# yazdayy/sound-event-detection

Measured on AMD Instinct MI355X. Metric: 10s@16kHz clips/sec (whole node) + ms/clip p50, Cnn_9_Gru_FrameAtt logmel, higher is better.
Workload: dtype f32 (conv2 of block 1 as Winograd F(4x4,3x3), blocks 2-4 as Winograd F(4x4,3x3): f32 transforms, f32 MFMA, f32 accumulate)

## Files before the change

sound-event-detection_amd/csrc/api.cpp:

```cpp
#include <new>
#include <hip/hip_runtime.h>

#include <algorithm>
#include <cmath>
#include <complex>
#include <cstdarg>
#include <cstdio>
#include <cstdlib>
#include <cstring>
#include <map>
#include <mutex>
#include <string>
#include <vector>

#include "../../include/sedx.h"
#include "rank.h"
#include "sedx_internal.h"

using namespace sedx;

struct EvSet {
  hipEvent_t ev[SEDX_N_STAGES + 1] = {};
  bool rec[SEDX_N_STAGES + 1] = {};
};
// ... 204 lines not shown
}

sedx_status run_body(sedx_handle* h, const ForwardPlan& p, float* ws, float* d_fw, float* d_clip, float* d_emb,
                     hipStream_t s) {
  const DevWeights& w = h->w;
  const Tuning& t = h->tune;
  const Geometry& g = p.g;
  const int64_t B = p.B;
  const int iB = (int)B, M = p.M, T3 = (int)g.Ts;
  float* X0 = ws + p.x0.off;
  float* A = ws + p.A.off;
  int* sched = reinterpret_cast<int*>(ws + p.sched.off);
  mark(h, 12, s);
  auto block1_first = [&]() {
    switch (p.block1) {
      case B1_CONV1C4_F43: launch_conv1_c4(X0, iB, (int)g.T, w.c1_w, w.c1_b, A, s); break;
      case B1_CONV1_F23:
      case B1_CONV1_F43: launch_conv1_nhwc(X0, iB, (int)g.T, w.c1_w, w.c1_b, A, s); break;
      case B1_PAD_EXACT:
      case B1_PAD_X3: launch_pad_x0(X0, iB, (int)g.T, A, s); break;
      case B1_F23_FUSED: break;
      case B1_VGG: launch_vgg_conv1(X0, iB, (int)g.T, w.c1_w, w.c1_b, A, s); break;
    }
  };
  if (p.claims) HIP_TRY(h, hipMemsetAsync(sched, 0, 7 * CONV_SCHED_INTS * sizeof(int), s));
  const bool first_early = t.pipelined && t.pipe_conv1_first;
  if (first_early) block1_first();
  if (t.pipelined && h->conv_done_recorded) HIP_TRY(h, hipStreamWaitEvent(s, h->conv_done, 0));
  mark(h, 1, s);
  capture(h, 0, X0, (size_t)B * g.T * 64, s);
  if (!first_early) block1_first();
// ... 19 lines not shown
      launch_conv3x3_deep(in, iB, c.T, c.F, c.cin, c.cout, w.wp[7] + deep_w_off(l), w.cb[7] + deep_b_off(l), out,
                          c.epi, p.c4 && l == 0, s);
      capture(h, i < 7 ? 2 + i : 40 + (i - 7), out, (size_t)B * c.To * c.Fo * c.cout, s);
      continue;
    }
    int* claim = p.claims ? sched + i * CONV_SCHED_INTS : nullptr;
    mark(h, 2 + i, s);
    WinoFamily wf;
    const bool wino = conv_launch_family(p, i, &wf);
    if (wino && wf == WINO_F23_BLOCK1)
      launch_block1_wino(in, iB, c.T, w.c1_w, w.c1_b, w.wu[k], w.cb[k], out, w.zero, w.trash, s, p.c4);
    else if (wino && wf == WINO_F23)
      launch_conv3x3_wino(in, iB, c.T, c.F, c.cin, c.cout, w.wu[k], w.cb[k], out, c.epi, w.zero, w.trash, s, c.order);
    else if (wino)
      launch_conv3x3_wino43(in, iB, c.T, c.F, c.cin, c.cout, w.wu43[k], w.cb[k], out, c.epi, w.trash, s, c.order,
                            p.c4, 0, claim);
    else if (i == 0 && p.block1 == B1_PAD_X3)
      launch_block1_fused_x3(nullptr, iB, c.T, in, w.c1_wt, w.c1_b, w.wx3[k], w.cb[k], out, claim, s);
    else if (i == 0)
      launch_block1_exact(in, iB, c.T, w.c1_w, w.c1_b, w.wp[k], w.cb[k], out, w.zero, s);
    else if (p.family == CONV_X3)
      launch_conv3x3_x3(in, iB, c.T, c.F, c.cin, c.cout, w.wx3[k], w.cb[k], out, c.epi, claim, s);
    else
      launch_conv3x3(in, iB, c.T, c.F, c.cin, c.cout, w.wp[k], w.cb[k], out, c.epi, w.zero, s);
    if (p.c4 && c.epi != EPI_FMEAN)
      capture_c4(h, 2 + i, out, B, c.To, c.Fo, c.cout, s);
    else
      capture(h, 2 + i, out, (size_t)B * c.To * c.Fo * c.cout, s);
  }
  mark(h, 9, s);
  if (t.pipelined) {
// ... 142 lines not shown
  h->cap_buf = d_buf;
  h->cap_bytes = bytes;
  return SEDX_OK;
}

sedx_status sedx_set_tuning(sedx_handle* h, int32_t knob, int32_t value) {
  if (!h) return SEDX_EINVAL;
  static const struct {
    int knob, lo, hi;
    int Tuning::*field;
  } knobs[] = {{SEDX_TUNE_GRU_KERNEL, SEDX_GRU_KERNEL_COOP, SEDX_GRU_KERNEL_PAIR, &Tuning::gru_kernel},
               {SEDX_TUNE_GRU_HANDOFF, SEDX_GRU_HANDOFF_AUTO, SEDX_GRU_HANDOFF_LOCAL, &Tuning::gru_handoff},
               {SEDX_TUNE_WINO_BLOCK1, 0, 2, &Tuning::wino_block1},
               {SEDX_TUNE_MEL_MFMA, 0, 1, &Tuning::mel_mfma},
               {SEDX_TUNE_GRU_SPIN, 0, INT32_MAX, &Tuning::gru_spin},
               {SEDX_TUNE_WINO_ORDER, 0, 2, &Tuning::wino_order},
               {SEDX_TUNE_GAMMA_SPEC, 0, 1, &Tuning::gamma_spec},
               {SEDX_TUNE_WINO_F43, 0, 2, &Tuning::wino_f43}};
  for (const auto& k : knobs) {
    if (k.knob != knob) continue;
    if (value < k.lo || value > k.hi) return fail(h, SEDX_EINVAL, "bad value %d for tuning knob %d", (int)value, (int)knob);
    h->tune.*k.field = value;
    return SEDX_OK;
  }
  return fail(h, SEDX_EINVAL, "unknown tuning knob %d", (int)knob);
}

sedx_status sedx_check_error(sedx_handle* h) {
  if (!h) return SEDX_EINVAL;
  return check_async_error(h);
}
// ... 584 lines not shown
```

sound-event-detection_amd/csrc/conv_wino.hip:

```cpp
#include <type_traits>

#include "sedx_internal.h"
#include "wino_geom.h"

namespace sedx {

typedef float f32x16 __attribute__((ext_vector_type(16)));
typedef float f32x4w __attribute__((ext_vector_type(4)));

#ifndef SEDX_WINO_ABL
#define SEDX_WINO_ABL 0
#endif
#ifndef SEDX_WINO_C1MFMA
#define SEDX_WINO_C1MFMA 0
#endif
#ifndef SEDX_WINO_VG
#define SEDX_WINO_VG 3
#endif
#ifndef SEDX_WINO_VG1
#define SEDX_WINO_VG1 9
#endif
#ifdef SEDX_WINO_STAMPS
__device__ unsigned long long g_wino_stamps[16];
#define WS_DECL                                      \
// ... 733 lines not shown
#pragma unroll
      for (int k = 0; k < 9; ++k) acc = fmaf(xv[k], s_w[(4 * cc + c) * 9 + k], acc);
      y[c] = fmaxf(acc + s_b[4 * cc + c], 0.0f);
    }
    *reinterpret_cast<float4*>(ob + (int64_t)cc * T * 256) = make_float4(y[0], y[1], y[2], y[3]);
  }
}

void launch_conv1_c4(const float* x0, int B, int T, const float* w1, const float* b1, float* out, hipStream_t s) {
  const int rb = (T + C1_ROWS - 1) / C1_ROWS;
  const int64_t blocks = (int64_t)B * rb;
  if (B <= 0 || T <= 0 || blocks > INT32_MAX || (int64_t)T * 64 > INT32_MAX) return note_launch_error(hipErrorInvalidValue);
  hipLaunchKernelGGL(conv1_c4_kernel, dim3((unsigned)blocks), dim3(256), 0, s, x0, T, rb, w1, b1, out);
}

#ifdef SEDX_WINO_STAMPS
void wino_stamps_rw(unsigned long long* h, bool reset) {
  if (reset) {
    static const unsigned long long z[16] = {};
    (void)hipMemcpyToSymbol(HIP_SYMBOL(g_wino_stamps), z, sizeof(z));
  } else {
    (void)hipMemcpyFromSymbol(h, HIP_SYMBOL(g_wino_stamps), 16 * sizeof(unsigned long long));
  }
}
#endif


}
```

sound-event-detection_amd/csrc/conv_wino43.hip:

```cpp
#include <type_traits>

#include "sedx_internal.h"
#include "wino_geom.h"

namespace sedx {

typedef float w43_f32x4 __attribute__((ext_vector_type(4)));

#ifndef SEDX_W43_ABL
#define SEDX_W43_ABL 0
#endif
#ifndef SEDX_W43_PRIO
#define SEDX_W43_PRIO 2
#endif
#ifndef SEDX_W43_USEL
#define SEDX_W43_USEL 1
#endif
#ifndef SEDX_W43_DMA_SPLIT
#define SEDX_W43_DMA_SPLIT 5
#endif

#ifdef SEDX_W43_STAMPS
__device__ unsigned long long g_w43_stamps[8];
#define W43_MARK(i)                                            \
  {                                                            \
    const unsigned long long n_ = __builtin_amdgcn_s_memtime(); \
    w43_st[i] += n_ - w43_t;                                   \
    w43_t = n_;                                                \
  }
#else
#define W43_MARK(i)
#endif

template <int N>
// ... 26 lines not shown
  v[1] = a + b;
  v[2] = a - b;
  const float c = e[4] - e[2], t = e[3] - e[1];
  v[3] = fmaf(2.0f, t, c);
  v[4] = fmaf(-2.0f, t, c);
  v[5] = fmaf(4.0f, e[1], fmaf(-5.0f, e[3], e[5]));
}
__device__ __forceinline__ void w43_at(const float (&m)[6], float (&z)[4]) {
  const float s12 = m[1] + m[2], d12 = m[1] - m[2], s34 = m[3] + m[4], d34 = m[3] - m[4];
  z[0] = (m[0] + s12) + s34;
  z[1] = fmaf(2.0f, d34, d12);
  z[2] = fmaf(4.0f, s34, s12);
  z[3] = fmaf(8.0f, d34, d12) + m[5];
}

template <int F, int EPI, int ROW, bool C4, int NT, int TG>
__device__ __forceinline__ void w43_body(const float* __restrict__ in, int B, int T, int Cin, int Cout,
                                         const float* __restrict__ U, int u_bytes, const float* __restrict__ bias,
                                         float* __restrict__ out, float* __restrict__ trash, int tb_per_clip,
                                         int ngroups, int order2d, int* __restrict__ sched, int wv) {
  using G = W43Geom<F, TG>;
  constexpr int RS = G::RS, PS = G::PS;
  static_assert(TG == 2 || (NT == 1 && (F == 16 || F == 8)), "16-tile items: 16-channel, F = 16 / 8 only");
  static_assert(NT == 4 || NT == 1, "channel tiles per item");
  using UF = typename std::conditional<NT == 4, w43_f32x4, float>::type;
  constexpr int VM = NT == 4 ? G::VM : TG == 2 ? 5 : 6;
  extern __shared__ __attribute__((aligned(16))) float smem[];

  const int lane = (int)__builtin_amdgcn_mbcnt_hi(~0u, __builtin_amdgcn_mbcnt_lo(~0u, 0u));
  const int tg = TG == 2 ? wv & 1 : 0;
  const int kk = lane >> 4, nn = lane & 15;

  auto decode = [&](int item, int& b_, int& t0_, int& g_) -> bool {
    const int xcd = item & 7, j = item >> 3;
    int jb, cgi;
    if constexpr (NT == 1) {
      const int tbl = B * tb_per_clip, gi = j / tbl, tb = j - gi * tbl;
      g_ = 8 * gi + xcd;
      if (g_ >= ngroups) return false;
      b_ = tb / tb_per_clip;
      t0_ = 4 * G::TRW * (tb - b_ * tb_per_clip);
// ... 42 lines not shown
    item = __builtin_amdgcn_readfirstlane(cl[1]);
  }
  if (!decode(item, b, t0, grp)) {
    claim_done();
    return;
  }

  const int tr = (F == 16 ? 4 * tg : F == 8 ? 8 * tg : F == 64 ? tg : 0) + nn / G::TFG;
  const int tf = (F == 32 ? 4 * tg : 0) + nn % G::TFG;

  const __amdgpu_buffer_rsrc_t r_in =
      __builtin_amdgcn_make_buffer_rsrc((void*)in, 0, (int)((int64_t)B * T * F * Cin * 4), 0x00020000);
  const __amdgpu_buffer_rsrc_t r_u = __builtin_amdgcn_make_buffer_rsrc((void*)U, 0, u_bytes, 0x00020000);
  const int nchunks = Cin / 4;
  auto halo_off = [&](int b_, int t0_) -> uint32_t {
    const int q = 64 * wv + lane;
    const int row = q / RS, col = q - (q / RS) * RS;
    const int t = t0_ - 1 + row, f = col - 1;
    const bool ok = row < G::RT && col < G::CS && t >= 0 && t < T && f >= 0 && f < F;
    if constexpr (C4)
      return ok ? (uint32_t)((((b_ * (Cin / 4) * T + t) * F + f) * 16)) : 0x80000000u;
    return ok ? (uint32_t)((((b_ * T + t) * F + f) * Cin) * 4) : 0x80000000u;
  };
  const uint32_t u_voff = 16 * lane + 1024 * wv;
  const uint32_t u_voff1 = wv < 9 ? u_voff : 0x80000000u;
  const uint32_t u_voff2 = wv + 6 < 9 ? u_voff + 6144 : 0x80000000u;
  const uint32_t bytes_per_chunk_u = 4 * G::USZ;
  auto dma_u_units = [&](int g_, int cc, int uslot, auto q0_tag, auto q1_tag) {
    if constexpr (SEDX_W43_ABL & 2) return;
    constexpr int Q0 = decltype(q0_tag)::value, Q1 = decltype(q1_tag)::value;
// ... 6 lines not shown
        if constexpr (TG == 1) w43_dma16(u_voff2, r_u, so, m0 + 6144);
      }
      return;
    }
    const uint32_t so = __builtin_amdgcn_readfirstlane((uint32_t)((g_ * nchunks + cc) * bytes_per_chunk_u));
    const uint32_t m0 = __builtin_amdgcn_readfirstlane(w43_lds_addr(smem + G::U_OFF + uslot * G::USZ + 256 * wv));
#pragma unroll
    for (int q = Q0; q < Q1; ++q) w43_dma16(u_voff, r_u, so + q * 12288, m0 + q * 12288);
  };
  auto dma_u = [&](int g_, int cc, int uslot) {
    dma_u_units(g_, cc, uslot, std::integral_constant<int, 0>{}, std::integral_constant<int, 3>{});
  };
  auto dma_h_planes = [&](uint32_t hof, int cc, int hslot, auto p0_tag, auto p1_tag) {
    if constexpr (SEDX_W43_ABL & 1) return;
    constexpr int P0 = decltype(p0_tag)::value, P1 = decltype(p1_tag)::value;
    const uint32_t so = __builtin_amdgcn_readfirstlane((uint32_t)(16 * (C4 ? cc * T * F : cc)));
    const bool tw = wv == G::HB;
    const uint32_t m0 = __builtin_amdgcn_readfirstlane(
        w43_lds_addr(tw ? smem + G::HTRASH_OFF : smem + G::H_OFF + hslot * G::HALO + 64 * wv));
    const uint32_t pstep = tw ? 0u : 4u * PS;
#pragma unroll
    for (int q = P0; q < P1; ++q) w43_dma4(hof, r_in, so + 4 * q, m0 + q * pstep);
  };
  auto dma_h = [&](uint32_t hof, int cc, int hslot) {
    dma_h_planes(hof, cc, hslot, std::integral_constant<int, 0>{}, std::integral_constant<int, 4>{});
  };

  constexpr int S = ROW >= 4 ? 0 : (EPI == EPI_STORE ? 4 : 1) * NT;
  float* const tr_lane = trash + (blockIdx.x & 31) * 256 + 4 * lane;
  auto opix = [&](int t, int f, int n, int To, int Fo) -> float* {
// ... 8 lines not shown
              __builtin_amdgcn_readfirstlane(w43_lds_addr(smem + G::BIAS_OFF + 256 * wv)));
  }
  uint32_t hof = halo_off(b, t0);
  dma_h(hof, 0, 0);
  dma_u(grp, 0, 0);
  dma_h(hof, 1, 1);
  dma_u(grp, 1, 1);
  dma_h(hof, 2, 2);
  if constexpr (S > 0) {
    float* const vt = tr_lane;
    const float zf = 0.0f;
#pragma unroll
    for (int i = 0; i < S; ++i) asm volatile("global_store_dword %0, %1, off" ::"v"(vt), "v"(zf) : "memory");
  }

  const int p_base = kk * PS + 4 * tr * RS + 4 * tf;
  constexpr int PA = ROW == 0 ? 4 : ROW == 5 ? 5 : ROW <= 2 ? 3 : 2;
  constexpr int PB = (ROW == 0 || ROW == 5) ? -1 : 4;
  constexpr int PC = ROW == 0 ? 2 : (ROW == 3 || ROW == 4 || ROW == 5) ? 3 : 2;
  constexpr int PD = ROW == 0 ? 0 : 1;
  constexpr float CC = ROW == 0 ? -5.0f : ROW == 1 ? -4.0f : ROW == 2 ? -4.0f : ROW == 3 ? 2.0f : ROW == 4 ? -2.0f : -5.0f;
  constexpr float CD = ROW == 0 ? 4.0f : ROW == 1 ? -4.0f : ROW == 2 ? 4.0f : ROW == 3 ? -2.0f : ROW == 4 ? 2.0f : 4.0f;
  typedef float f2v __attribute__((ext_vector_type(2)));
  auto read_row = [](uint32_t a, auto r_tag, f2v (&x)[3]) {
    constexpr int R = decltype(r_tag)::value;
    asm volatile("ds_read_b64 %0, %1 offset:%2" : "=v"(x[0]) : "v"(a), "n"(4 * (R * RS)));
    asm volatile("ds_read_b64 %0, %1 offset:%2" : "=v"(x[1]) : "v"(a), "n"(4 * (R * RS + 2)));
    asm volatile("ds_read_b64 %0, %1 offset:%2" : "=v"(x[2]) : "v"(a), "n"(4 * (R * RS + 4)));
  };
  auto read_u = [](uint32_t a, auto j_tag, UF& u) {
    constexpr int J = decltype(j_tag)::value;
// ... 384 lines not shown
            for (int j = 0; j < 4; ++j) {
              const int tj = 4 * j + ((le >> 2) & 3);
              const int trj = (F == 16 ? 4 * tg : F == 8 ? 8 * tg : F == 64 ? tg : 0) + tj / G::TFG;
              const int tfj = (F == 32 ? 4 * tg : 0) + tj % G::TFG;
              const int t = 4 * (t0 / 4 + trj) + ROW, f = 4 * tfj + (le & 3);
              float* dst = t < T ? opix(t, f, n, T, F) : tr_lane;
              if constexpr (SEDX_W43_ABL & 16) dst = tr_lane;
              *reinterpret_cast<w43_f32x4*>(dst) = ost2[j];
            }
          }
        } else {
          if (E2 || (q & 1)) {
            float* dst;
            if constexpr (EPI == EPI_POOL2) {
              const int to = 2 * trg + (ROW >> 1), fo = 2 * tf + (ROW & 1);
              dst = to < T / 2 ? opix(to, fo, n, T / 2, F / 2) : tr_lane;
              if constexpr (SEDX_W43_ABL & 32) dst = tr_lane;
            } else {
              const int t = 4 * trg + ROW;
              dst = (t < T && !(tf & 1)) ? out + (int64_t)(b * T + t) * Cout + n : tr_lane;
            }
            *reinterpret_cast<w43_f32x4*>(dst) = ost[nt];
          }
        }
      }
    }
    W43_MARK(2)
#ifdef SEDX_W43_STAMPS
    w43_st[4] += 1;
#endif
    if (!has_next) break;
// ... 1 lines not shown
    b = nb_;
    t0 = nt0;
    grp = ng;
    hof = nhof;
  }
  claim_done();
#ifdef SEDX_W43_STAMPS
  if (lane == 0 && (blockIdx.x & 15) == 0) {
    w43_st[3] = __builtin_amdgcn_s_memtime() - w43_t0;
    for (int i = 0; i < 5; ++i) atomicAdd(&g_w43_stamps[i], w43_st[i]);
    atomicAdd(&g_w43_stamps[5], 1ull);
  }
#endif
}

#define SEDX_W43_ROWS(F_, EPI_, C4_, NT_, TG_, ...)                         \
  switch (TG_ == 2 ? wv >> 1 : wv) {                                       \
    case 0: w43_body<F_, EPI_, 0, C4_, NT_, TG_>(__VA_ARGS__); break;      \
    case 1: w43_body<F_, EPI_, 1, C4_, NT_, TG_>(__VA_ARGS__); break;      \
    case 2: w43_body<F_, EPI_, 2, C4_, NT_, TG_>(__VA_ARGS__); break;      \
    case 3: w43_body<F_, EPI_, 3, C4_, NT_, TG_>(__VA_ARGS__); break;      \
    case 4: w43_body<F_, EPI_, 4, C4_, NT_, TG_>(__VA_ARGS__); break;      \
    default: w43_body<F_, EPI_, 5, C4_, NT_, TG_>(__VA_ARGS__); break;     \
  }

template <int F, int EPI, bool C4, int NT = 4, int TG = 2>
__global__ __launch_bounds__(384 * TG, 1) void conv3x3_wino43_kernel(const float* __restrict__ in, int B, int T, int Cin,
                                                                int Cout, const float* __restrict__ U, int u_bytes,
                                                                const float* __restrict__ bias, float* __restrict__ out,
                                                                float* __restrict__ trash, int tb_per_clip,
                                                                int ngroups, int order2d, int* __restrict__ sched) {
  const int wv = __builtin_amdgcn_readfirstlane((int)threadIdx.x >> 6);
#if SEDX_W43_PRIO == 1
  if (wv >= 8) __builtin_amdgcn_s_setprio(1);
#elif SEDX_W43_PRIO == 2
  if (wv >= 8) __builtin_amdgcn_s_setprio(2);
  else if (wv >= 4) __builtin_amdgcn_s_setprio(1);
#elif SEDX_W43_PRIO == 3
  if (wv < 4) __builtin_amdgcn_s_setprio(2);
  else if (wv < 8) __builtin_amdgcn_s_setprio(1);
#endif
#ifdef SEDX_W43_DELAY
  if ((blockIdx.x & 1) && blockIdx.x < 256) {
    const unsigned long long t0_ = __builtin_amdgcn_s_memtime();
    while (__builtin_amdgcn_s_memtime() - t0_ < (unsigned long long)SEDX_W43_DELAY) __builtin_amdgcn_s_sleep(8);
  }
#endif
  SEDX_W43_ROWS(F, EPI, C4, NT, TG, in, B, T, Cin, Cout, U, u_bytes, bias, out, trash, tb_per_clip, ngroups, order2d,
                sched, wv)
}
#undef SEDX_W43_ROWS

template <int F, int TG>
static void launch_w43_g(const ConvLaunch& p, const float* in, int T, int Cin, int Cout, const float* U,
                         const float* bias, float* out, int epi, float* trash, bool c4, int* sched, hipStream_t s) {
  using G = W43Geom<F, TG>;
  const int u_bytes = 2 * Cin * Cout * 36 * 4;
  int* const sched_k = p.claim ? sched : nullptr;
#define SEDX_W43_LAUNCH(E)                                                                                  \
  {                                                                                                         \
    auto* k_ = conv3x3_wino43_kernel<F, E, true, 1, TG>;    \
    if constexpr (TG == 2)                                                                                  \
      k_ = p.NT == 1 ? (c4 ? conv3x3_wino43_kernel<F, E, true, 1> : conv3x3_wino43_kernel<F, E, false, 1>)  \
                     : (c4 ? conv3x3_wino43_kernel<F, E, true, 4> : conv3x3_wino43_kernel<F, E, false, 4>); \
    if (!launch_info(reinterpret_cast<const void*>(k_), G::THREADS, G::LDS_BYTES, c4).ok) return;           \
    hipLaunchKernelGGL(k_, dim3((unsigned)p.nwg), dim3(G::THREADS), G::LDS_BYTES, s, in, p.clips, T, Cin,   \
                       Cout, U, u_bytes, bias, out, trash, p.tb_per_clip, p.ngroups, p.order2d, sched_k);   \
    return;                                                                                                 \
  }
  if constexpr (F == 64) {
    if (epi == EPI_POOL2) SEDX_W43_LAUNCH(EPI_POOL2);
  } else if constexpr (F == 8) {
    if (epi == EPI_STORE) SEDX_W43_LAUNCH(EPI_STORE);
    if (epi == EPI_FMEAN) SEDX_W43_LAUNCH(EPI_FMEAN);
  } else {
    if (epi == EPI_STORE) SEDX_W43_LAUNCH(EPI_STORE);
    if (epi == EPI_POOL2) SEDX_W43_LAUNCH(EPI_POOL2);
  }
#undef SEDX_W43_LAUNCH
  note_launch_error(hipErrorInvalidValue);
}

template <int F>
static void launch_w43_f(const ConvLaunch& p, const float* in, int T, int Cin, int Cout, const float* U,
                         const float* bias, float* out, int epi, float* trash, bool c4, int* sched, hipStream_t s) {
  if constexpr (F == 16 || F == 8) {
    if (p.TG == 1) return launch_w43_g<F, 1>(p, in, T, Cin, Cout, U, bias, out, epi, trash, c4, sched, s);
  }
  launch_w43_g<F, 2>(p, in, T, Cin, Cout, U, bias, out, epi, trash, c4, sched, s);
}

void launch_conv3x3_wino43(const float* in, int B, int T, int F, int Cin, int Cout, const float* U43,
                           const float* bias, float* out, int epi, float* trash, hipStream_t s, int order, bool c4,
                           int nt_force, int* sched) {
  do {
    const ConvLaunch p = plan_conv_launch(WINO_F43, device_cus(), B, T, F, Cin, Cout, epi, order, c4, nt_force,
                                          sched != nullptr);
    if (p.reject) return note_launch_error(hipErrorInvalidValue);
    switch (F) {
      case 64: launch_w43_f<64>(p, in, T, Cin, Cout, U43, bias, out, epi, trash, c4, sched, s); break;
      case 32: launch_w43_f<32>(p, in, T, Cin, Cout, U43, bias, out, epi, trash, c4, sched, s); break;
      case 16: launch_w43_f<16>(p, in, T, Cin, Cout, U43, bias, out, epi, trash, c4, sched, s); break;
      default: launch_w43_f<8>(p, in, T, Cin, Cout, U43, bias, out, epi, trash, c4, sched, s); break;
    }
    in += p.clips * p.in_clip, out += p.clips * p.out_clip, B -= p.clips;
  } while (B > 0);
}

#ifdef SEDX_W43_STAMPS
void w43_stamps_rw(unsigned long long* h, bool reset) {
  if (reset) {
    static const unsigned long long z[8] = {};
    (void)hipMemcpyToSymbol(HIP_SYMBOL(g_w43_stamps), z, sizeof(z));
  } else {
    (void)hipMemcpyFromSymbol(h, HIP_SYMBOL(g_w43_stamps), 8 * sizeof(unsigned long long));
  }
}
#endif
// ... 25 lines not shown
```

sound-event-detection_amd/csrc/plan.cpp:

```cpp
#include "plan.h"

#include "wino_geom.h"

#include <algorithm>
#include <cmath>
#include <cstdio>

namespace sedx {

Geometry geometry_from_T(const Model& m, int64_t T) {
  Geometry g;
  g.T = T;
  g.T1 = T / 2;
  g.T2 = g.T1 / 2;
  g.T3 = g.T2 / 2;
  g.T4 = g.T3 / 2;
  g.T5 = g.T4 / 2;
  if (m.vgg) {
    g.Ts = g.T4;
    g.rep = m.head == HEAD_ATT ? VGG_ATT_REPEAT : g.Ts >= 1 && g.Ts <= VGG_OUT_FRAMES ? (int)(VGG_OUT_FRAMES / g.Ts) : 1;
    g.fw_len = g.rep * g.Ts;
    g.out_frames = VGG_OUT_FRAMES;
    return g;
  }
// ... 29 lines not shown
const char* plan_forward(const Model& m, const Tuning& t, int64_t B, int64_t T, ForwardPlan* p) {
  const Geometry g = geometry_from_T(m, T);
  p->g = g;
  p->B = B;
  p->M = (int)(B * g.Ts);
  const bool deep = m.depth == 14;
  p->nlayers = m.vgg ? VGG_LAYERS - 1 : deep ? 11 : 7;
  p->first_deep = m.vgg ? p->nlayers : deep ? 6 : 7;
  const bool wino = t.precision == SEDX_PRECISION_WINOGRAD, x3 = t.precision == SEDX_PRECISION_X3;
  if (x3) p->block1 = B1_PAD_X3;
  else if (!wino || t.wino_block1 == 0) p->block1 = B1_PAD_EXACT;
  else if (t.wino_f43 == 2) p->block1 = t.wino_block1 == 2 ? B1_CONV1C4_F43 : B1_CONV1_F43;
  else p->block1 = t.wino_block1 == 2 ? B1_F23_FUSED : B1_CONV1_F23;
  p->family = x3 ? CONV_X3 : !wino ? CONV_EXACT : t.wino_f43 ? CONV_WINO43 : CONV_WINO;
  p->c4 = wino && t.wino_f43 && t.wino_block1 == 2;
  p->claims = x3 || (p->family == CONV_WINO43 && B >= 8);
  if (m.vgg) p->block1 = B1_VGG, p->family = CONV_EXACT, p->c4 = false, p->claims = false;
  static const int variant[8] = {2, -1, 0, 1, 3, 3, 4, 5};
  p->gru_variant = variant[t.gru_kernel];
  p->gru_fast = t.gru_handoff == SEDX_GRU_HANDOFF_AUTO || t.gru_handoff == SEDX_GRU_HANDOFF_LOCAL;
  p->gru_spread = t.gru_handoff == SEDX_GRU_HANDOFF_SPREAD || (t.gru_handoff == SEDX_GRU_HANDOFF_AUTO && t.pipelined);
  size_t end = 0;
  p->x0 = take(end, (size_t)B * T * 64);
  const size_t a0 = end;
  size_t a_conv = p->block1 == B1_VGG                                   ? (size_t)B * g.T1 * 32 * 64
                  : p->block1 == B1_F23_FUSED                           ? 0
                  : p->block1 == B1_PAD_EXACT || p->block1 == B1_PAD_X3 ? block1_pad_floats((int)B, (int)T)
                                                                         : (size_t)B * T * 64 * 64;
  size_t p_conv = 0;
  const int64_t Ts[4] = {g.T, g.T1, g.T2, g.T3};
  for (int i = 6; i < p->nlayers; ++i) {
    const int blk = (i + 1) / 2, cout = 64 << blk, F = 64 >> blk, last = i == 10, pool = i % 2 == 0 && !last;
// ... 4 lines not shown
    ext = std::max(ext, (size_t)B * p->layers[i].To * p->layers[i].Fo * cout);
  }
  for (int i = 0; m.vgg && i < p->nlayers; ++i) {
    const int l = i + 1, cout = VGG_COUT[l], blk = (i + 1) / 2, F = 32 >> blk, last = i == 4, pool = i % 2 == 0;
    const int Tl = (int)(blk == 0 ? g.T1 : blk == 1 ? g.T2 : g.T3);
    p->layers[i] = ConvLayer{Tl, F, VGG_CIN[l], cout, last ? EPI_MAXPOOL2_FMEAN : pool ? EPI_MAXPOOL2 : EPI_STORE,
                             pool ? Tl / 2 : Tl, last ? 1 : pool ? F / 2 : F, 0, 0, 0};
    size_t& ext = i % 2 ? a_conv : p_conv;
    ext = std::max(ext, (size_t)B * p->layers[i].To * p->layers[i].Fo * cout);
  }
  for (int i = 0; !m.vgg && i < (deep ? 6 : 7); ++i) {
    const int blk = (i + 1) / 2, cout = 64 << blk, Tl = (int)Ts[blk], F = 64 >> blk, pool = i % 2 == 0 && i < 6;
    p->layers[i] = ConvLayer{Tl, F, i == 0 ? 64 : i % 2 ? cout / 2 : cout, cout,
                             i == 6 ? EPI_FMEAN : pool ? EPI_POOL2 : EPI_STORE,
                             pool ? Tl / 2 : Tl, i == 6 ? 1 : pool ? F / 2 : F, 0, 0,
                             i == 0 && p->block1 == B1_CONV1_F23 ? 0 : t.wino_order};
    size_t& ext = i % 2 ? a_conv : p_conv;
    ext = std::max(ext, (size_t)B * p->layers[i].To * p->layers[i].Fo * cout);
  }
  const size_t M = (size_t)p->M;
  size_t e_head = a0;
  p->G = take(e_head, m.decision ? 0 : M * (deep && m.seq == SEQ_GRU ? 6144 : 1536));
  p->Hs = take(e_head, M * (deep ? 2048 : 512));
  p->O = take(e_head, m.decision ? 0 : M * 512);
  p->LG = take(e_head, M * m.nac);
  p->gru = take(e_head, deep ? 0 : gru_coop_workspace_bytes((int)B) / 4);
  size_t e_a = std::max(a0 + align256(a_conv * 4), e_head);
  if (m.seq == SEQ_CONFORMER) {
    size_t e_cf = a0;
    p->X = take(e_cf, M * CF_D);
    p->Xn = take(e_cf, M * CF_D);
// ... 266 lines not shown
```

sound-event-detection_amd/csrc/plan.h:

```cpp
#pragma once
#include <cstddef>
#include <cstdint>
#include <vector>

#include "../../include/sedx.h"
#include "weights.h"

namespace sedx {

constexpr size_t align256(size_t bytes) { return (bytes + 255) & ~size_t(255); }
inline size_t carve(size_t& end, size_t bytes) {
  const size_t at = end;
  end = at + align256(bytes);
  return at;
}

enum ConvEpi { EPI_STORE = 0, EPI_POOL2 = 1, EPI_FMEAN = 2, EPI_MAXPOOL2 = 3, EPI_MAXPOOL2_FMEAN = 4 };
constexpr int CONV_SCHED_INTS = 256;
constexpr size_t block1_pad_floats(int B, int T) { return (size_t)B * (T + 2) * 66; }
constexpr size_t gru_coop_workspace_bytes(int ) { return 10240 + (size_t)8 * 2 * 32 * 256 * 4; }

struct Geometry {
  int64_t T, T1, T2, T3, fw_len, out_frames;
  int64_t T4 = 0, T5 = 0, Ts = 0;
// ... 38 lines not shown
constexpr int MAX_CONV_LAYERS = 11;
struct ConvLayer {
  int T, F, cin, cout, epi;
  int To, Fo;
  size_t in, out;
  int order;
};
struct ForwardPlan {
  Geometry g{};
  int64_t B = 0;
  int M = 0;
  int nlayers = 7, first_deep = 7;
  Block1Form block1 = B1_PAD_EXACT;
  ConvFamily family = CONV_EXACT;
  bool c4 = false;
  bool claims = false;
  ConvLayer layers[MAX_CONV_LAYERS] = {};
  int gru_variant = 2;
  bool gru_fast = false, gru_spread = false;
  Region x0, A, P, sched;
  Region G, Hs, O, LG, gru;
  Region X, Xn, Hb, AV, Rr, RK;
  size_t total_bytes = 0;
  char reject[96] = {};
};
const char* plan_forward(const Model& m, const Tuning& t, int64_t B, int64_t T, ForwardPlan* p);

enum WinoFamily { WINO_F23 = SEDX_CONV_F23, WINO_F23_BLOCK1 = SEDX_CONV_F23_BLOCK1, WINO_F43 = SEDX_CONV_F43 };
struct ConvLaunch {
  const char* reject = nullptr;
// ... 70 lines not shown
```

sound-event-detection_amd/csrc/sedx_internal.h:

```cpp
#pragma once
#include <hip/hip_runtime.h>

#include <cstdio>
#include <cstdlib>
#include <map>
#include <mutex>
#include <stdint.h>

#include <algorithm>
#include <utility>
#include <vector>

#include "../../include/sedx.h"
#include "plan.h"
#include "weights.h"

namespace sedx {

struct FrontendParams {
  const float* audio;
  const int16_t* audio_i16;
  int64_t clip_stride;
  int32_t n_clips;
  int32_t n_win;
// ... 47 lines not shown
void launch_conv3x3(const float* in, int B, int T, int F, int Cin, int Cout,
                    const float* wp, const float* bias, float* out, int epi,
                    const float* zero16, hipStream_t s);

void launch_vgg_conv1(const float* x, int B, int T, const float* w1, const float* b1, float* out, hipStream_t s);
void launch_vgg_att_head(const float* logits, int B, int T, int C, int ldl, int out_frames, int ratio,
                         float* framewise, float* clipwise, float* emb_cla, hipStream_t s);
void launch_vgg_fc_head(const float* logits, int B, int T, int C, int ldl, int out_frames, int ratio,
                        float* framewise, float* clipwise, hipStream_t s);

void launch_conv3x3_wino(const float* in, int B, int T, int F, int Cin, int Cout,
                         const float* U, const float* bias, float* out, int epi,
                         const float* zero16, float* trash, hipStream_t s, int order = 0);
void launch_conv3x3_wino43(const float* in, int B, int T, int F, int Cin, int Cout, const float* U43,
                           const float* bias, float* out, int epi, float* trash, hipStream_t s, int order = 0,
                           bool c4 = false, int nt_force = 0, int* sched = nullptr);
void launch_conv3x3_deep(const float* in, int B, int T, int F, int Cin, int Cout, const float* wd,
                         const float* bias, float* out, int epi, bool in_c4, hipStream_t s);
void launch_c4_to_nhwc(const float* src, int B, int T, int F, int C, float* dst, hipStream_t s);
void launch_block1_wino(const float* x0, int B, int T, const float* w1, const float* b1, const float* U,
                        const float* bias, float* out, const float* zero16, float* trash, hipStream_t s,
                        bool c4 = false);
void launch_conv1_nhwc(const float* x0, int B, int T, const float* w1, const float* b1, float* out,
                       hipStream_t s);
void launch_conv1_c4(const float* x0, int B, int T, const float* w1, const float* b1, float* out, hipStream_t s);

inline thread_local hipError_t t_launch_err = hipSuccess;
inline void note_launch_error(hipError_t e) {
  if (e != hipSuccess && t_launch_err == hipSuccess) t_launch_err = e;
}
inline hipError_t take_launch_error() {
  const hipError_t e = t_launch_err;
  t_launch_err = hipSuccess;
  return e;
}


struct LaunchInfo {
  bool ok = false;
  int ncu = 0;
// ... 170 lines not shown
```

sound-event-detection_amd/csrc/wino_geom.h:

```cpp
#pragma once

namespace sedx {

template <int F, int TG, int NT = 2, bool C1 = false>
struct WinoGeom {
  static constexpr int WAVES = 4 * TG;
  static constexpr int THREADS = 64 * WAVES;
  static constexpr int NCH = 32 * NT;
  static constexpr int P = 32 * TG;
  static constexpr int FT = F / 2;
  static constexpr int TRW = P / FT;
  static constexpr int RT = 2 * TRW + 2, CS = F + 2, KC = 4;
  static constexpr int PL = RT * CS;
  static constexpr int PLP = (PL + 63) / 64 * 64;
  static constexpr int A_SZ = KC * (C1 && PLP < 64 * WAVES ? 64 * WAVES : PLP);
  static constexpr int W_SZ = 16 * KC * NCH;
  static constexpr int BUF = A_SZ + W_SZ;
#ifndef SEDX_WINO_NBUF
#define SEDX_WINO_NBUF 3
#endif
  static constexpr int NBUF = SEDX_WINO_NBUF;
  static constexpr int UW = W_SZ / 256;
  static constexpr int UA = C1 ? 0 : PLP / 64;
  static constexpr int U = UW + UA;
// ... 11 lines not shown
  static constexpr int WG_PER_CU = WAVES == 8 || LDS_BYTES > 80 * 1024 ? 1 : 2;
  static_assert(NT == 1 || NT == 2, "channel tiles per wave");
  static_assert(P % FT == 0, "whole tile rows per workgroup");
  static_assert(VM_MIN * (NBUF - 1) <= 63, "vmcnt field");
  static_assert(LDS_BYTES <= 160 * 1024, "LDS per workgroup");
  static_assert(!C1 || (F == 64 && NT == 2 && PLP <= 64 * WAVES && UX <= WAVES && NBUF >= 3), "C1: block 1 (64 bins), a conv1 group per wave");
};

#ifndef SEDX_W43_EPI2
#define SEDX_W43_EPI2 0
#endif
#ifndef SEDX_W43_CLAIM
#define SEDX_W43_CLAIM 1
#endif

template <int F, int TG = 2>
struct W43Geom {
  static constexpr int WAVES = 6 * TG, THREADS = 64 * WAVES;
  static constexpr int NT = 4, NCH = 64;
  static constexpr int TILES = 16 * TG;
  static constexpr int FT = F / 4;
  static constexpr int TRW = TILES / FT;
  static constexpr int TFG = F == 8 ? 2 : F == 64 ? 16 : 4;
  static constexpr int TRG = 16 / TFG;
  static constexpr int RT = 4 * TRW + 2, CS = F + 2;
  static constexpr int RS = F == 64 ? 66 : F == 32 ? 36 : F == 16 ? 20 : 10;
  static constexpr int HB = TG == 2 ? 11 : 6;
  static constexpr int PS = 64 * HB + 2;
  static constexpr int HALO = 4 * PS;
  static constexpr int USZ1 = 36 * 4 * 16;
  static constexpr int NB = 3;
  static constexpr int XRS = 4 * 80;
  static constexpr int XTG = 6 * 2 * XRS;
  static constexpr int USZ = TG == 2 ? 36 * 4 * NCH : (USZ1 > XTG ? USZ1 : XTG);
  static constexpr int U_OFF = 0, H_OFF = NB * USZ, BIAS_OFF = H_OFF + NB * HALO, BIAS_MAX = 512;
  static constexpr int HTRASH_OFF = BIAS_OFF + BIAS_MAX;
  static constexpr int X2_OFF = HTRASH_OFF + 64, X2 = SEDX_W43_EPI2 && TG == 2 ? 3072 : 0;
  static constexpr int CL_OFF = X2_OFF + X2;
  static constexpr int LDS_BYTES = 4 * (CL_OFF + (SEDX_W43_CLAIM ? 4 : 0));
  static constexpr int VM = 7;

  static_assert(F == 64 || F == 32 || F == 16 || F == 8, "F");
  static_assert(RT * RS <= 64 * HB, "halo plane fits its DMA blocks");
  static_assert(TG == 1 || TG == 2, "TG");
  static_assert(TG == 1 ? HB == WAVES : HB == WAVES - 1, "halo blocks: one per wave (TG 2: wave 11 trash)");
  static_assert(TG == 1 || 36 % WAVES == 0, "U units per wave");
  static_assert(TG * XTG <= USZ, "the tile groups' exchange fits one U slot");
  static_assert(LDS_BYTES <= 160 * 1024, "LDS per workgroup");
  static_assert(FT * TRW == TILES && TFG * TRG == 16, "tile groups");
};

}
```

Measured before the change: 13800.

## Emit block-1 conv1 in planar layout and DMA 16-byte halo rows into Winograd F43

Adds a conv1 kernel that writes its output as per-channel planes (B, C, T, 64) instead of the chunk-of-4 layout. Adds a planar-input variant of the F(4x4,3x3) Winograd kernel for block 1's conv2, which loads halo planes with 16-byte DMA pieces of 4 bins, using a wider row stride and fewer DMA waves. The aim is fewer and wider global loads for the halo fill of the most expensive conv layer. The planar path becomes the default for the conv1c4+F43 block-1 form, and wino_order=3 opts back out to the old path. Out-of-range pooled outputs are redirected to a trash buffer.

```diff
diff --git a/sound-event-detection_amd/csrc/api.cpp b/sound-event-detection_amd/csrc/api.cpp
--- a/sound-event-detection_amd/csrc/api.cpp
+++ b/sound-event-detection_amd/csrc/api.cpp
@@ -242,7 +242,10 @@
   mark(h, 12, s);
   auto block1_first = [&]() {
     switch (p.block1) {
-      case B1_CONV1C4_F43: launch_conv1_c4(X0, iB, (int)g.T, w.c1_w, w.c1_b, A, s); break;
+      case B1_CONV1C4_F43:
+        if (p.b1_planar) launch_conv1_planar(X0, iB, (int)g.T, w.c1_w, w.c1_b, A, s);
+        else launch_conv1_c4(X0, iB, (int)g.T, w.c1_w, w.c1_b, A, s);
+        break;
       case B1_CONV1_F23:
       case B1_CONV1_F43: launch_conv1_nhwc(X0, iB, (int)g.T, w.c1_w, w.c1_b, A, s); break;
       case B1_PAD_EXACT:
@@ -292,7 +295,7 @@
       launch_conv3x3_wino(in, iB, c.T, c.F, c.cin, c.cout, w.wu[k], w.cb[k], out, c.epi, w.zero, w.trash, s, c.order);
     else if (wino)
       launch_conv3x3_wino43(in, iB, c.T, c.F, c.cin, c.cout, w.wu43[k], w.cb[k], out, c.epi, w.trash, s, c.order,
-                            p.c4, 0, claim);
+                            p.c4, 0, claim, i == 0 && p.b1_planar);
     else if (i == 0 && p.block1 == B1_PAD_X3)
       launch_block1_fused_x3(nullptr, iB, c.T, in, w.c1_wt, w.c1_b, w.wx3[k], w.cb[k], out, claim, s);
     else if (i == 0)
@@ -465,7 +468,7 @@
                {SEDX_TUNE_WINO_BLOCK1, 0, 2, &Tuning::wino_block1},
                {SEDX_TUNE_MEL_MFMA, 0, 1, &Tuning::mel_mfma},
                {SEDX_TUNE_GRU_SPIN, 0, INT32_MAX, &Tuning::gru_spin},
-               {SEDX_TUNE_WINO_ORDER, 0, 2, &Tuning::wino_order},
+               {SEDX_TUNE_WINO_ORDER, 0, 3, &Tuning::wino_order},
                {SEDX_TUNE_GAMMA_SPEC, 0, 1, &Tuning::gamma_spec},
                {SEDX_TUNE_WINO_F43, 0, 2, &Tuning::wino_f43}};
   for (const auto& k : knobs) {
diff --git a/sound-event-detection_amd/csrc/conv_wino.hip b/sound-event-detection_amd/csrc/conv_wino.hip
--- a/sound-event-detection_amd/csrc/conv_wino.hip
+++ b/sound-event-detection_amd/csrc/conv_wino.hip
@@ -771,6 +771,54 @@
   hipLaunchKernelGGL(conv1_c4_kernel, dim3((unsigned)blocks), dim3(256), 0, s, x0, T, rb, w1, b1, out);
 }
 
+__global__ __launch_bounds__(256) void conv1_planar_kernel(const float* __restrict__ x0, int T, int rb_per_clip,
+                                                           const float* __restrict__ w1, const float* __restrict__ b1,
+                                                           float* __restrict__ out) {
+  __shared__ float s_w[64 * 9], s_b[64];
+  __shared__ float s_x[C1_ROWS + 2][66];
+  const int b = blockIdx.x / rb_per_clip;
+  const int t0 = (blockIdx.x - b * rb_per_clip) * C1_ROWS;
+  for (int i = threadIdx.x; i < 64 * 9; i += 256) s_w[i] = w1[i];
+  if (threadIdx.x < 64) s_b[threadIdx.x] = b1[threadIdx.x];
+  const float* xb = x0 + (int64_t)b * T * 64;
+  for (int i = threadIdx.x; i < (C1_ROWS + 2) * 66; i += 256) {
+    const int r = i / 66, c = i - r * 66;
+    const int t = t0 - 1 + r, f = c - 1;
+    s_x[r][c] = (t >= 0 && t < T && f >= 0 && f < 64) ? xb[t * 64 + f] : 0.0f;
+  }
+  __syncthreads();
+  static_assert(C1_ROWS * 16 == 64, "a wave covers the rows' 4-bin groups");
+  const int lane = threadIdx.x & 63, cq = threadIdx.x >> 6;
+  const int r = lane >> 4, f0 = 4 * (lane & 15);
+  if (t0 + r >= T) return;
+  float xv[3][6];
+#pragma unroll
+  for (int dy = 0; dy < 3; ++dy)
+#pragma unroll
+    for (int dx = 0; dx < 6; ++dx) xv[dy][dx] = s_x[r + dy][f0 + dx];
+  float* ob = out + (((int64_t)b * 64 + 16 * cq) * T + t0 + r) * 64 + f0;
+  for (int c = 0; c < 16; ++c) {
+    const float* wc = s_w + (16 * cq + c) * 9;
+    const float bc = s_b[16 * cq + c];
+    float y[4];
+#pragma unroll
+    for (int p = 0; p < 4; ++p) {
+      float acc = 0.0f;
+#pragma unroll
+      for (int k = 0; k < 9; ++k) acc = fmaf(xv[k / 3][p + k % 3], wc[k], acc);
+      y[p] = fmaxf(acc + bc, 0.0f);
+    }
+    *reinterpret_cast<float4*>(ob + (int64_t)c * T * 64) = make_float4(y[0], y[1], y[2], y[3]);
+  }
+}
+
+void launch_conv1_planar(const float* x0, int B, int T, const float* w1, const float* b1, float* out, hipStream_t s) {
+  const int rb = (T + C1_ROWS - 1) / C1_ROWS;
+  const int64_t blocks = (int64_t)B * rb;
+  if (B <= 0 || T <= 0 || blocks > INT32_MAX || (int64_t)T * 64 > INT32_MAX) return note_launch_error(hipErrorInvalidValue);
+  hipLaunchKernelGGL(conv1_planar_kernel, dim3((unsigned)blocks), dim3(256), 0, s, x0, T, rb, w1, b1, out);
+}
+
 #ifdef SEDX_WINO_STAMPS
 void wino_stamps_rw(unsigned long long* h, bool reset) {
   if (reset) {
diff --git a/sound-event-detection_amd/csrc/conv_wino43.hip b/sound-event-detection_amd/csrc/conv_wino43.hip
--- a/sound-event-detection_amd/csrc/conv_wino43.hip
+++ b/sound-event-detection_amd/csrc/conv_wino43.hip
@@ -18,6 +18,9 @@
 #endif
 #ifndef SEDX_W43_DMA_SPLIT
 #define SEDX_W43_DMA_SPLIT 5
+#endif
+#ifndef SEDX_W43_PL_AT
+#define SEDX_W43_PL_AT 0
 #endif
 
 #ifdef SEDX_W43_STAMPS
@@ -74,17 +77,18 @@
   z[3] = fmaf(8.0f, d34, d12) + m[5];
 }
 
-template <int F, int EPI, int ROW, bool C4, int NT, int TG>
+template <int F, int EPI, int ROW, bool C4, int NT, int TG, bool PL = false>
 __device__ __forceinline__ void w43_body(const float* __restrict__ in, int B, int T, int Cin, int Cout,
                                          const float* __restrict__ U, int u_bytes, const float* __restrict__ bias,
                                          float* __restrict__ out, float* __restrict__ trash, int tb_per_clip,
                                          int ngroups, int order2d, int* __restrict__ sched, int wv) {
-  using G = W43Geom<F, TG>;
+  using G = W43Geom<F, TG, PL>;
   constexpr int RS = G::RS, PS = G::PS;
   static_assert(TG == 2 || (NT == 1 && (F == 16 || F == 8)), "16-tile items: 16-channel, F = 16 / 8 only");
   static_assert(NT == 4 || NT == 1, "channel tiles per item");
+  static_assert(!PL || (C4 && F == 64 && TG == 2), "planar input: block 1's conv2, chunk-of-4 output");
   using UF = typename std::conditional<NT == 4, w43_f32x4, float>::type;
-  constexpr int VM = NT == 4 ? G::VM : TG == 2 ? 5 : 6;
+  constexpr int VM = NT == 4 ? G::VM : PL ? 2 : TG == 2 ? 5 : 6;
   extern __shared__ __attribute__((aligned(16))) float smem[];
 
   const int lane = (int)__builtin_amdgcn_mbcnt_hi(~0u, __builtin_amdgcn_mbcnt_lo(~0u, 0u));
@@ -157,6 +161,15 @@
   const __amdgpu_buffer_rsrc_t r_u = __builtin_amdgcn_make_buffer_rsrc((void*)U, 0, u_bytes, 0x00020000);
   const int nchunks = Cin / 4;
   auto halo_off = [&](int b_, int t0_) -> uint32_t {
+    if constexpr (PL) {
+      int l_ = lane;
+      asm volatile("" : "+v"(l_));
+      const int q = 64 * (wv % 3) + l_;
+      const int row = q / 18, g = q - (q / 18) * 18;
+      const int t = t0_ - 1 + row;
+      const bool ok = row < G::RT && g >= 1 && g <= 16 && t >= 0 && t < T;
+      return ok ? (uint32_t)((((b_ * Cin * T + t) * F + 4 * (g - 1)) * 4)) : 0x80000000u;
+    }
     const int q = 64 * wv + lane;
     const int row = q / RS, col = q - (q / RS) * RS;
     const int t = t0_ - 1 + row, f = col - 1;
@@ -193,6 +206,16 @@
   auto dma_h_planes = [&](uint32_t hof, int cc, int hslot, auto p0_tag, auto p1_tag) {
     if constexpr (SEDX_W43_ABL & 1) return;
     constexpr int P0 = decltype(p0_tag)::value, P1 = decltype(p1_tag)::value;
+    if constexpr (PL) {
+      if constexpr (P0 <= SEDX_W43_PL_AT && SEDX_W43_PL_AT < P1) {
+        const int k = wv / 3;
+        const uint32_t so = __builtin_amdgcn_readfirstlane((uint32_t)((4 * cc + k) * T * F * 4));
+        const uint32_t m0 = __builtin_amdgcn_readfirstlane(
+            w43_lds_addr(smem + G::H_OFF + hslot * G::HALO + k * PS + 1 + 256 * (wv - 3 * k)));
+        w43_dma16(hof, r_in, so, m0);
+      }
+      return;
+    }
     const uint32_t so = __builtin_amdgcn_readfirstlane((uint32_t)(16 * (C4 ? cc * T * F : cc)));
     const bool tw = wv == G::HB;
     const uint32_t m0 = __builtin_amdgcn_readfirstlane(
@@ -231,7 +254,7 @@
     for (int i = 0; i < S; ++i) asm volatile("global_store_dword %0, %1, off" ::"v"(vt), "v"(zf) : "memory");
   }
 
-  const int p_base = kk * PS + 4 * tr * RS + 4 * tf;
+  const int p_base = kk * PS + 4 * tr * RS + 4 * tf + (PL ? 4 : 0);
   constexpr int PA = ROW == 0 ? 4 : ROW == 5 ? 5 : ROW <= 2 ? 3 : 2;
   constexpr int PB = (ROW == 0 || ROW == 5) ? -1 : 4;
   constexpr int PC = ROW == 0 ? 2 : (ROW == 3 || ROW == 4 || ROW == 5) ? 3 : 2;
@@ -646,7 +669,8 @@
             float* dst;
             if constexpr (EPI == EPI_POOL2) {
               const int to = 2 * trg + (ROW >> 1), fo = 2 * tf + (ROW & 1);
-              dst = to < T / 2 ? opix(to, fo, n, T / 2, F / 2) : tr_lane;
+              dst = to < T / 2 ? opix(to, fo, n, T / 2, F / 2)
+                               : (PL ? trash + (blockIdx.x & 31) * 256 + 4 * le : tr_lane);
               if constexpr (SEDX_W43_ABL & 32) dst = tr_lane;
             } else {
               const int t = 4 * trg + ROW;
@@ -678,22 +702,21 @@
 #endif
 }
 
-#define SEDX_W43_ROWS(F_, EPI_, C4_, NT_, TG_, ...)                         \
+#define SEDX_W43_ROWS(F_, EPI_, C4_, NT_, TG_, PL_, ...)                    \
   switch (TG_ == 2 ? wv >> 1 : wv) {                                       \
-    case 0: w43_body<F_, EPI_, 0, C4_, NT_, TG_>(__VA_ARGS__); break;      \
-    case 1: w43_body<F_, EPI_, 1, C4_, NT_, TG_>(__VA_ARGS__); break;      \
-    case 2: w43_body<F_, EPI_, 2, C4_, NT_, TG_>(__VA_ARGS__); break;      \
-    case 3: w43_body<F_, EPI_, 3, C4_, NT_, TG_>(__VA_ARGS__); break;      \
-    case 4: w43_body<F_, EPI_, 4, C4_, NT_, TG_>(__VA_ARGS__); break;      \
-    default: w43_body<F_, EPI_, 5, C4_, NT_, TG_>(__VA_ARGS__); break;     \
-  }
-
-template <int F, int EPI, bool C4, int NT = 4, int TG = 2>
-__global__ __launch_bounds__(384 * TG, 1) void conv3x3_wino43_kernel(const float* __restrict__ in, int B, int T, int Cin,
-                                                                int Cout, const float* __restrict__ U, int u_bytes,
-                                                                const float* __restrict__ bias, float* __restrict__ out,
-                                                                float* __restrict__ trash, int tb_per_clip,
-                                                                int ngroups, int order2d, int* __restrict__ sched) {
+    case 0: w43_body<F_, EPI_, 0, C4_, NT_, TG_, PL_>(__VA_ARGS__); break; \
+    case 1: w43_body<F_, EPI_, 1, C4_, NT_, TG_, PL_>(__VA_ARGS__); break; \
+    case 2: w43_body<F_, EPI_, 2, C4_, NT_, TG_, PL_>(__VA_ARGS__); break; \
+    case 3: w43_body<F_, EPI_, 3, C4_, NT_, TG_, PL_>(__VA_ARGS__); break; \
+    case 4: w43_body<F_, EPI_, 4, C4_, NT_, TG_, PL_>(__VA_ARGS__); break; \
+    default: w43_body<F_, EPI_, 5, C4_, NT_, TG_, PL_>(__VA_ARGS__); break; \
+  }
+
+template <int F, int EPI, bool C4, int NT, int TG, bool PL>
+__device__ __forceinline__ void w43_entry(const float* __restrict__ in, int B, int T, int Cin, int Cout,
+                                          const float* __restrict__ U, int u_bytes, const float* __restrict__ bias,
+                                          float* __restrict__ out, float* __restrict__ trash, int tb_per_clip,
+                                          int ngroups, int order2d, int* __restrict__ sched) {
   const int wv = __builtin_amdgcn_readfirstlane((int)threadIdx.x >> 6);
 #if SEDX_W43_PRIO == 1
   if (wv >= 8) __builtin_amdgcn_s_setprio(1);
@@ -710,17 +733,52 @@
     while (__builtin_amdgcn_s_memtime() - t0_ < (unsigned long long)SEDX_W43_DELAY) __builtin_amdgcn_s_sleep(8);
   }
 #endif
-  SEDX_W43_ROWS(F, EPI, C4, NT, TG, in, B, T, Cin, Cout, U, u_bytes, bias, out, trash, tb_per_clip, ngroups, order2d,
+  SEDX_W43_ROWS(F, EPI, C4, NT, TG, PL, in, B, T, Cin, Cout, U, u_bytes, bias, out, trash, tb_per_clip, ngroups, order2d,
                 sched, wv)
 }
 #undef SEDX_W43_ROWS
+
+template <int F, int EPI, bool C4, int NT = 4, int TG = 2>
+__global__ __launch_bounds__(384 * TG, 1) void conv3x3_wino43_kernel(const float* __restrict__ in, int B, int T, int Cin,
+                                                                int Cout, const float* __restrict__ U, int u_bytes,
+                                                                const float* __restrict__ bias, float* __restrict__ out,
+                                                                float* __restrict__ trash, int tb_per_clip,
+                                                                int ngroups, int order2d, int* __restrict__ sched) {
+  w43_entry<F, EPI, C4, NT, TG, false>(in, B, T, Cin, Cout, U, u_bytes, bias, out, trash, tb_per_clip, ngroups, order2d,
+                                       sched);
+}
+
+template <int NT>
+__global__ __launch_bounds__(768, 1) void conv3x3_wino43_planar_kernel(const float* __restrict__ in, int B, int T,
+                                                                   int Cin, int Cout, const float* __restrict__ U,
+                                                                   int u_bytes, const float* __restrict__ bias,
+                                                                   float* __restrict__ out, float* __restrict__ trash,
+                                                                   int tb_per_clip, int ngroups, int order2d,
+                                                                   int* __restrict__ sched) {
+  w43_entry<64, EPI_POOL2, true, NT, 2, true>(in, B, T, Cin, Cout, U, u_bytes, bias, out, trash, tb_per_clip, ngroups,
+                                              order2d, sched);
+}
 
 template <int F, int TG>
 static void launch_w43_g(const ConvLaunch& p, const float* in, int T, int Cin, int Cout, const float* U,
-                         const float* bias, float* out, int epi, float* trash, bool c4, int* sched, hipStream_t s) {
+                         const float* bias, float* out, int epi, float* trash, bool c4, bool planar, int* sched,
+                         hipStream_t s) {
   using G = W43Geom<F, TG>;
   const int u_bytes = 2 * Cin * Cout * 36 * 4;
   int* const sched_k = p.claim ? sched : nullptr;
+  if (planar) {
+    if constexpr (F == 64 && TG == 2) {
+      using GP = W43Geom<64, 2, true>;
+      if (c4 && epi == EPI_POOL2) {
+        auto* k_ = p.NT == 1 ? conv3x3_wino43_planar_kernel<1> : conv3x3_wino43_planar_kernel<4>;
+        if (!launch_info(reinterpret_cast<const void*>(k_), GP::THREADS, GP::LDS_BYTES, true).ok) return;
+        hipLaunchKernelGGL(k_, dim3((unsigned)p.nwg), dim3(GP::THREADS), GP::LDS_BYTES, s, in, p.clips, T, Cin, Cout, U,
+                           u_bytes, bias, out, trash, p.tb_per_clip, p.ngroups, p.order2d, sched_k);
+        return;
+      }
+    }
+    return note_launch_error(hipErrorInvalidValue);
+  }
 #define SEDX_W43_LAUNCH(E)                                                                                  \
   {                                                                                                         \
     auto* k_ = conv3x3_wino43_kernel<F, E, true, 1, TG>;    \
@@ -747,25 +805,26 @@
 
 template <int F>
 static void launch_w43_f(const ConvLaunch& p, const float* in, int T, int Cin, int Cout, const float* U,
-                         const float* bias, float* out, int epi, float* trash, bool c4, int* sched, hipStream_t s) {
+                         const float* bias, float* out, int epi, float* trash, bool c4, bool planar, int* sched,
+                         hipStream_t s) {
   if constexpr (F == 16 || F == 8) {
-    if (p.TG == 1) return launch_w43_g<F, 1>(p, in, T, Cin, Cout, U, bias, out, epi, trash, c4, sched, s);
-  }
-  launch_w43_g<F, 2>(p, in, T, Cin, Cout, U, bias, out, epi, trash, c4, sched, s);
+    if (p.TG == 1) return launch_w43_g<F, 1>(p, in, T, Cin, Cout, U, bias, out, epi, trash, c4, planar, sched, s);
+  }
+  launch_w43_g<F, 2>(p, in, T, Cin, Cout, U, bias, out, epi, trash, c4, planar, sched, s);
 }
 
 void launch_conv3x3_wino43(const float* in, int B, int T, int F, int Cin, int Cout, const float* U43,
                            const float* bias, float* out, int epi, float* trash, hipStream_t s, int order, bool c4,
-                           int nt_force, int* sched) {
+                           int nt_force, int* sched, bool planar_in) {
   do {
     const ConvLaunch p = plan_conv_launch(WINO_F43, device_cus(), B, T, F, Cin, Cout, epi, order, c4, nt_force,
                                           sched != nullptr);
     if (p.reject) return note_launch_error(hipErrorInvalidValue);
     switch (F) {
-      case 64: launch_w43_f<64>(p, in, T, Cin, Cout, U43, bias, out, epi, trash, c4, sched, s); break;
-      case 32: launch_w43_f<32>(p, in, T, Cin, Cout, U43, bias, out, epi, trash, c4, sched, s); break;
-      case 16: launch_w43_f<16>(p, in, T, Cin, Cout, U43, bias, out, epi, trash, c4, sched, s); break;
-      default: launch_w43_f<8>(p, in, T, Cin, Cout, U43, bias, out, epi, trash, c4, sched, s); break;
+      case 64: launch_w43_f<64>(p, in, T, Cin, Cout, U43, bias, out, epi, trash, c4, planar_in, sched, s); break;
+      case 32: launch_w43_f<32>(p, in, T, Cin, Cout, U43, bias, out, epi, trash, c4, planar_in, sched, s); break;
+      case 16: launch_w43_f<16>(p, in, T, Cin, Cout, U43, bias, out, epi, trash, c4, planar_in, sched, s); break;
+      default: launch_w43_f<8>(p, in, T, Cin, Cout, U43, bias, out, epi, trash, c4, planar_in, sched, s); break;
     }
     in += p.clips * p.in_clip, out += p.clips * p.out_clip, B -= p.clips;
   } while (B > 0);
diff --git a/sound-event-detection_amd/csrc/plan.cpp b/sound-event-detection_amd/csrc/plan.cpp
--- a/sound-event-detection_amd/csrc/plan.cpp
+++ b/sound-event-detection_amd/csrc/plan.cpp
@@ -67,8 +67,10 @@
   else p->block1 = t.wino_block1 == 2 ? B1_F23_FUSED : B1_CONV1_F23;
   p->family = x3 ? CONV_X3 : !wino ? CONV_EXACT : t.wino_f43 ? CONV_WINO43 : CONV_WINO;
   p->c4 = wino && t.wino_f43 && t.wino_block1 == 2;
+  p->b1_planar = p->block1 == B1_CONV1C4_F43 && t.wino_order != 3;
+  const int wino_order = t.wino_order == 3 ? 1 : t.wino_order;
   p->claims = x3 || (p->family == CONV_WINO43 && B >= 8);
-  if (m.vgg) p->block1 = B1_VGG, p->family = CONV_EXACT, p->c4 = false, p->claims = false;
+  if (m.vgg) p->block1 = B1_VGG, p->family = CONV_EXACT, p->c4 = false, p->b1_planar = false, p->claims = false;
   static const int variant[8] = {2, -1, 0, 1, 3, 3, 4, 5};
   p->gru_variant = variant[t.gru_kernel];
   p->gru_fast = t.gru_handoff == SEDX_GRU_HANDOFF_AUTO || t.gru_handoff == SEDX_GRU_HANDOFF_LOCAL;
@@ -103,7 +105,7 @@
     p->layers[i] = ConvLayer{Tl, F, i == 0 ? 64 : i % 2 ? cout / 2 : cout, cout,
                              i == 6 ? EPI_FMEAN : pool ? EPI_POOL2 : EPI_STORE,
                              pool ? Tl / 2 : Tl, i == 6 ? 1 : pool ? F / 2 : F, 0, 0,
-                             i == 0 && p->block1 == B1_CONV1_F23 ? 0 : t.wino_order};
+                             i == 0 && p->block1 == B1_CONV1_F23 ? 0 : wino_order};
     size_t& ext = i % 2 ? a_conv : p_conv;
     ext = std::max(ext, (size_t)B * p->layers[i].To * p->layers[i].Fo * cout);
   }
diff --git a/sound-event-detection_amd/csrc/plan.h b/sound-event-detection_amd/csrc/plan.h
--- a/sound-event-detection_amd/csrc/plan.h
+++ b/sound-event-detection_amd/csrc/plan.h
@@ -76,6 +76,7 @@
   Block1Form block1 = B1_PAD_EXACT;
   ConvFamily family = CONV_EXACT;
   bool c4 = false;
+  bool b1_planar = false;
   bool claims = false;
   ConvLayer layers[MAX_CONV_LAYERS] = {};
   int gru_variant = 2;
diff --git a/sound-event-detection_amd/csrc/sedx_internal.h b/sound-event-detection_amd/csrc/sedx_internal.h
--- a/sound-event-detection_amd/csrc/sedx_internal.h
+++ b/sound-event-detection_amd/csrc/sedx_internal.h
@@ -85,7 +85,7 @@
                          const float* zero16, float* trash, hipStream_t s, int order = 0);
 void launch_conv3x3_wino43(const float* in, int B, int T, int F, int Cin, int Cout, const float* U43,
                            const float* bias, float* out, int epi, float* trash, hipStream_t s, int order = 0,
-                           bool c4 = false, int nt_force = 0, int* sched = nullptr);
+                           bool c4 = false, int nt_force = 0, int* sched = nullptr, bool planar_in = false);
 void launch_conv3x3_deep(const float* in, int B, int T, int F, int Cin, int Cout, const float* wd,
                          const float* bias, float* out, int epi, bool in_c4, hipStream_t s);
 void launch_c4_to_nhwc(const float* src, int B, int T, int F, int C, float* dst, hipStream_t s);
@@ -95,6 +95,7 @@
 void launch_conv1_nhwc(const float* x0, int B, int T, const float* w1, const float* b1, float* out,
                        hipStream_t s);
 void launch_conv1_c4(const float* x0, int B, int T, const float* w1, const float* b1, float* out, hipStream_t s);
+void launch_conv1_planar(const float* x0, int B, int T, const float* w1, const float* b1, float* out, hipStream_t s);
 
 inline thread_local hipError_t t_launch_err = hipSuccess;
 inline void note_launch_error(hipError_t e) {
diff --git a/sound-event-detection_amd/csrc/wino_geom.h b/sound-event-detection_amd/csrc/wino_geom.h
--- a/sound-event-detection_amd/csrc/wino_geom.h
+++ b/sound-event-detection_amd/csrc/wino_geom.h
@@ -49,7 +49,7 @@
 #define SEDX_W43_CLAIM 1
 #endif
 
-template <int F, int TG = 2>
+template <int F, int TG = 2, bool PL = false>
 struct W43Geom {
   static constexpr int WAVES = 6 * TG, THREADS = 64 * WAVES;
   static constexpr int NT = 4, NCH = 64;
@@ -59,9 +59,9 @@
   static constexpr int TFG = F == 8 ? 2 : F == 64 ? 16 : 4;
   static constexpr int TRG = 16 / TFG;
   static constexpr int RT = 4 * TRW + 2, CS = F + 2;
-  static constexpr int RS = F == 64 ? 66 : F == 32 ? 36 : F == 16 ? 20 : 10;
+  static constexpr int RS = PL ? 72 : F == 64 ? 66 : F == 32 ? 36 : F == 16 ? 20 : 10;
   static constexpr int HB = TG == 2 ? 11 : 6;
-  static constexpr int PS = 64 * HB + 2;
+  static constexpr int PS = PL ? 3 * 256 + 2 : 64 * HB + 2;
   static constexpr int HALO = 4 * PS;
   static constexpr int USZ1 = 36 * 4 * 16;
   static constexpr int NB = 3;
@@ -73,10 +73,12 @@
   static constexpr int X2_OFF = HTRASH_OFF + 64, X2 = SEDX_W43_EPI2 && TG == 2 ? 3072 : 0;
   static constexpr int CL_OFF = X2_OFF + X2;
   static constexpr int LDS_BYTES = 4 * (CL_OFF + (SEDX_W43_CLAIM ? 4 : 0));
-  static constexpr int VM = 7;
+  static constexpr int VM = PL ? 4 : 7;
 
   static_assert(F == 64 || F == 32 || F == 16 || F == 8, "F");
-  static_assert(RT * RS <= 64 * HB, "halo plane fits its DMA blocks");
+  static_assert(PL ? RT * RS <= 3 * 256 && 1 + 3 * 256 <= PS : RT * RS <= 64 * HB, "halo plane fits its DMA blocks");
+  static_assert(!PL || (F == 64 && TG == 2 && WAVES == 12 && RS == 4 * 18), "planar input: block 1, four planes x three pieces");
+  static_assert(PS % 4 == 2 && PS >= RT * RS, "plane stride");
   static_assert(TG == 1 || TG == 2, "TG");
   static_assert(TG == 1 ? HB == WAVES : HB == WAVES - 1, "halo blocks: one per wave (TG 2: wave 11 trash)");
   static_assert(TG == 1 || 36 % WAVES == 0, "U units per wave");
```

New measurement: 13950, median of 6. 1.1% higher.
